# rgovindjee/mpconstellation

Measured on AMD Instinct MI355X. Metric: satellite-MPC-steps/sec (whole constellation; 1 step = discretize + constraint terms + solve per SCP iteration; inputs and results resident in HBM -- value_pcie is the same step with H2D of the inputs and D2H of the results inside), higher is better.
Workload: dtype f64

## Files before the change

mpconstellation_amd/csrc/solve_driver.hpp:

```cpp
#pragma once

#ifdef MPCX_WS_LDS
extern __shared__ double mpcx_ws_lds[];
#endif

namespace MPCX_NS {
#ifdef MPCX_PHASE_TIMING
#define PT_DECL unsigned long long pt_[12] = {0,0,0,0,0,0,0,0,0,0,0,0}, pt0_ = 0; unsigned pc_[12] = {0,0,0,0,0,0,0,0,0,0,0,0}; \
    const unsigned long long rt0_ = __builtin_amdgcn_s_memrealtime(), mt0_ = __builtin_amdgcn_s_memtime();
#define PT_BEGIN pt0_ = __builtin_amdgcn_s_memtime();
#define PT_END(i) { pt_[i] += __builtin_amdgcn_s_memtime() - pt0_; pc_[i]++; }
#else
#define PT_DECL
#define PT_BEGIN
#define PT_END(i)
#endif

#ifndef MPCX_SOLVE_WAVES
#define MPCX_SOLVE_WAVES 2
#endif

#ifndef MPCX_TP
__shared__ SatData g_sd;
__shared__ Scratch g_w;
// ... 65 lines not shown
    double v[GR_N];
    gr_clear(v);
    v[0] = r.sq; v[1] = r.zsum; v[2] = r.lsum; v[3] = r.prod_sum; v[4] = r.g_tf;
    v[GR_SUM] = r.dual_max; v[GR_SUM + 1] = r.prim_max; v[GR_SUM + 2] = r.prod_max;
    v[GR_SUM + GR_MAX] = r.prod_min;
    grid_reduce(g, v, lane);
    r.sq = v[0]; r.zsum = v[1]; r.lsum = v[2]; r.prod_sum = v[3]; r.g_tf = v[4];
    r.dual_max = v[GR_SUM]; r.prim_max = v[GR_SUM + 1]; r.prod_max = v[GR_SUM + 2]; r.prod_min = v[GR_SUM + GR_MAX];
    const double gtf = 1.0 + r.g_tf - gz[0] + gz[1];
    r.dual_max = fmax(r.dual_max, fabs(gtf)); r.sq += gtf * gtf;
    const double gv[2] = {-tf - b_tf[0], tf - b_tf[1]};
#pragma unroll
    for (int j = 0; j < 2; ++j) {
        const double pr = gv[j] + gs[j], sz = gs[j] * gz[j], q = sz - mu;
        r.prim_max = fmax(r.prim_max, fabs(pr)); r.sq += pr * pr + q * q;
        r.zsum += fabs(gz[j]); r.prod_min = fmin(r.prod_min, sz); r.prod_max = fmax(r.prod_max, sz); r.prod_sum += sz;
    }
}

template <bool SHARED>
__device__ __forceinline__ void solve_satellite(const SolveArgs &a, const int sat, const int slot, SatData &sd, Scratch &w, const int lane, GridSync *gsync = nullptr)
{
    PT_DECL
    const int Kmax = a.K;
    const int K = uni(a.Ks ? a.Ks[sat] : Kmax);
    if (K < 3 || K > Kmax) {
        cgf64 *xb = (cgf64 *)a.xbar + (size_t)sat * 7 * Kmax, *ub = (cgf64 *)a.ubar + (size_t)sat * 3 * Kmax;
        for (int e = lane; e < 7 * Kmax; e += 64) { a.X[(size_t)sat * 7 * Kmax + e] = xb[e]; a.NU[(size_t)sat * 7 * Kmax + e] = 0.0; }
        for (int e = lane; e < 3 * Kmax; e += 64) a.U[(size_t)sat * 3 * Kmax + e] = ub[e];
        if (lane == 0) {
            a.tf_out[sat] = (a.o.fixed_tf && !SHARED) ? 0.0 : a.tfbar[sat];
            a.status[sat] = MPCX_ST_BADK; a.iters[sat] = 0; a.kkt[sat] = 0.0;
            if (a.nreg) { a.nreg[2 * sat] = 0; a.nreg[2 * sat + 1] = -1; }
        }
        return;
    }
    { const Sat sv = sat_view(a, sat, slot, K, Kmax); if (lane == 0) g_s = sv; }
    WG_SYNC();
    Sat &s = g_s;
    const int KP = uni(s.KP);
    const SolveOpts &o = a.o;

    PT_BEGIN
    if (lane == 0) {
        double xK[7];
        for (int i = 0; i < 7; ++i) xK[i] = s.xbar[(size_t)i * Kmax + K - 1];
        build_terminal(xK, a.consts[(size_t)sat * MPCX_NCONST + MPCX_C_MU], a.r_des[sat], o, sd);
        sd.tfbar = a.tfbar[sat];
        double x0[3];
        for (int i = 0; i < 3; ++i) x0[i] = s.xbar[(size_t)i * Kmax];
        sd.infeas = structural_violation(x0, K, sd);
#ifdef MPCX_PHASE_TIMING
        for (int i = 0; i < 16; ++i) sd.fpt[i] = 0;
#endif
    }
    WG_SYNC();
    PT_END(11)
    PT_BEGIN
    double gr[GR_N];
    if (SHARED) {
        gr_clear(gr);
        gr[GR_SUM] = fmax(sd.infeas, -(sd.b_tf[0] + sd.b_tf[1]));
        grid_reduce(*gsync, gr, lane);
        if (lane == 0) sd.infeas = gsync->aborted ? 1.0 : gr[GR_SUM];
        WG_SYNC();
    }
    if (sd.infeas > 0.0) {
        for (int e = lane; e < 7 * Kmax; e += 64) { a.X[(size_t)sat * 7 * Kmax + e] = s.xbar[e]; a.NU[(size_t)sat * 7 * Kmax + e] = 0.0; }
        for (int e = lane; e < 3 * Kmax; e += 64) a.U[(size_t)sat * 3 * Kmax + e] = s.ubar[e];
        if (lane == 0) {
            if (!sd.fixed_tf || SHARED) a.tf_out[sat] = sd.tfbar; else a.tf_out[sat] = 0.0;
            a.status[sat] = (SHARED && gsync->aborted) ? MPCX_ST_NUMERIC : MPCX_ST_INFEASIBLE; a.iters[sat] = 0; a.kkt[sat] = sd.infeas;
            if (a.nreg) { a.nreg[2 * sat] = 0; a.nreg[2 * sat + 1] = -1; }
        }
        return;
    }
    {
        double *stg = (double *)&w;
        static_assert(sizeof(Scratch) >= 16 * MPCX_STAGE_DOUBLES * sizeof(double), "stage transposition buffer");
        for (int k0 = 0; k0 < K - 1; k0 += 16) {
            const int nk = (K - 1 - k0 < 16) ? K - 1 - k0 : 16;
            cgf64 *rec = s.A(k0);
            for (int e = lane; e < nk * MPCX_STAGE_DOUBLES; e += 64) stg[e] = rec[e];
            WG_SYNC();
            for (int e = lane; e < 16 * MPCX_STAGE_DOUBLES; e += 64) {
                const int f = e >> 4, kl = e & 15;
                if (kl < nk) s.stT[f * KP + k0 + kl] = stg[kl * MPCX_STAGE_DOUBLES + f];
            }
            WG_SYNC();
        }
    }
    PT_END(9)
    PT_BEGIN
    bool pushed = false;
    for (int k = lane; k < K; k += 64) {
        double x[7], u[3];
        for (int i = 0; i < 7; ++i) x[i] = s.xbar[(size_t)i * s.ldk + k];
        for (int i = 0; i < 3; ++i) u[i] = s.ubar[(size_t)i * s.ldk + k];
        const double rn = sqrt(x[0] * x[0] + x[1] * x[1] + x[2] * x[2]);
        const auto rb = s.rbn(k);
        for (int i = 0; i < 3; ++i) rb[i] = x[i] / rn;
        const auto p = s.itn(k);
        for (int i = 0; i < 7; ++i) { p[I_NU + i] = 0.0; p[I_LAM + i] = 0.0; }
        if (k == K - 1) for (int i = 0; i < 7; ++i) p[I_T + i] = 0.0;
        for (int i = 0; i < 7; ++i) p[I_X + i] = x[i];
        for (int i = 0; i < 3; ++i) p[I_U + i] = u[i];
// ... 276 lines not shown
            if (dec && cen) { have_trial = 1; break; }
            alpha = uni(alpha * 0.5);
        }
        if (!have_trial) {
            PT_BEGIN
            eval_residual<true>(s, sd, alpha, mu, mu_clip, lane);
            PT_END(10)
            if (SHARED) shared_trial();
        }
#ifdef MPCX_ITER_LOG
        if (lane == 0 && 5 * iter + 4 < 7 * K) { double *lg = a.X + (size_t)sat * 7 * Kmax + 5 * iter; lg[0] = mu; lg[1] = E0; lg[2] = alpha; lg[3] = delta_w; lg[4] = (double)fail_mask; }
#endif
        n_small = (alpha < kFbAlpha) ? n_small + 1 : 0;
        if (lane == 0) { wf64 *q = s.it; s.it = s.itB; s.itB = q; lf64 *g = s.itg; s.itg = s.itgB; s.itgB = g; }
        WG_SYNC();
        if (SHARED) { gs[0] = gst[0]; gs[1] = gst[1]; gz[0] = gzt[0]; gz[1] = gzt[1]; }
        {
            const double sq0 = rt.sq + 2.0 * mu * rt.prod_sum - (double)nzc * mu * mu;
            const ResAcc t = rt;
            WG_SYNC();
            r0 = t; r0.sq = sq0;
            WG_SYNC();
        }
    }

    for (int k = lane; k < K; k += 64) {
        const auto p = s.itn(k);
        for (int i = 0; i < 7; ++i) {
#ifndef MPCX_ITER_LOG
            a.X[(size_t)sat * 7 * Kmax + (size_t)i * Kmax + k] = p[I_X + i];
#endif
#if !(defined(MPCX_ITER_LOG) && defined(MPCX_LOG_IT))
            a.NU[(size_t)sat * 7 * Kmax + (size_t)i * Kmax + k] = (k <= K - 2) ? p[I_NU + i] : 0.0;
#endif
        }
#ifndef MPCX_ITER_LOG
        for (int i = 0; i < 3; ++i) a.U[(size_t)sat * 3 * Kmax + (size_t)i * Kmax + k] = p[I_U + i];
#endif
    }
    for (int k = K + lane; k < Kmax; k += 64) {
        for (int i = 0; i < 7; ++i) { a.X[(size_t)sat * 7 * Kmax + (size_t)i * Kmax + k] = 0.0; a.NU[(size_t)sat * 7 * Kmax + (size_t)i * Kmax + k] = 0.0; }
        for (int i = 0; i < 3; ++i) a.U[(size_t)sat * 3 * Kmax + (size_t)i * Kmax + k] = 0.0;
    }
    if (lane == 0) {
        a.tf_out[sat] = (sd.fixed_tf && !SHARED) ? r0.g_tf : s.itg[G_TF];
        a.status[sat] = status;
        a.iters[sat] = it_count;
        a.kkt[sat] = E0;
        if (a.nreg) { a.nreg[2 * sat] = n_reg; a.nreg[2 * sat + 1] = first_reg; }
#ifdef MPCX_PHASE_TIMING
        double *dbg = a.NU + (size_t)sat * 7 * Kmax;
        for (int i = 0; i < 12; ++i) { dbg[2 * i] = (double)pt_[i]; dbg[2 * i + 1] = (double)pc_[i]; }
        for (int i = 0; i < 16; ++i) dbg[24 + i] = (double)sd.fpt[i];
        dbg[40] = (double)(__builtin_amdgcn_s_memrealtime() - rt0_); dbg[41] = (double)(__builtin_amdgcn_s_memtime() - mt0_);
#ifdef MPCX_TP
        for (int i = 0; i < 16; ++i) dbg[48 + i] = (double)s.mail[16 + i];
#endif
#endif
    }
}

}
```

mpconstellation_amd/csrc/solve_phases.hpp:

```cpp
#pragma once

namespace MPCX_NS {
#ifdef MPCX_TWO_WAVE
using namespace mpcx;
#endif

struct ResAcc {
    double dual_max, prim_max, sq, zsum, lsum, prod_min, prod_max, prod_sum;
    double g_tf;
};

struct SatData {
    double aT[8][7], bT[8];
    int nT, linvt;
    int fixed_tf;
    int shared;
    double tS, rS;
    double w_vt, gh_vt, zeta_vt;
    double b_u, b_rmax, b_rmin, b_rfmax, b_tf[2], vt_des, w_tr, w_nu, tfbar;
    double WxK[49];
    double WxKsoft[49], gxKsoft[7];
    double ta[NTERM][7], tw[NTERM], tgh[NTERM], twin[NTERM];
    double avt[7], Hv[36], cv, gam, Wtf, gtf, sigmax;
    double Mb[NBD][NBD];
    double Sb[NBD][NBD];
    double siglam[NCH], xK[NCH][7];
    double sol[NBD];
    double zeta[NTERM];
    double red[8];
    double gl[3][GL_N];
    ResAcc racc[2];
    double rs_gtf, rs_rvt, rs_gex[NTERM];
    int dir_finite;
    struct Drv {
        double mu, dw_last, E0, delta_w, alpha, tau, mu_cur, rn0, mu_clip;
        int n_acc, status, it_count, n_reg, first_reg, mono, refined_prev, n_small, iter, have_dir, have_trial, clean, ls;
    } dv;
    double infeas;
    int flag;
#ifdef MPCX_PHASE_TIMING
    unsigned long long fpt[16];
#endif
};

__device__ __forceinline__ double relax(double b) { return b + kBoundRelax * fmax(1.0, fabs(b)); }

__device__ __forceinline__ double wave_max(double v)
{
#pragma unroll
    for (int o = 32; o > 0; o >>= 1) v = fmax(v, __shfl_xor(v, o, 64));
    return v;
}
__device__ __forceinline__ double wave_min(double v)
{
#pragma unroll
    for (int o = 32; o > 0; o >>= 1) v = fmin(v, __shfl_xor(v, o, 64));
    return v;
}
__device__ __forceinline__ double wave_sum(double v)
{
#pragma unroll
    for (int o = 32; o > 0; o >>= 1) v += __shfl_xor(v, o, 64);
    return v;
}

__device__ __forceinline__ double gshfl8(double v, int q)
{
    switch (q) {
    case 0: return bcast8<0>(v);
    case 1: return bcast8<1>(v);
    case 2: return bcast8<2>(v);
    case 3: return bcast8<3>(v);
    case 4: return bcast8<4>(v);
    case 5: return bcast8<5>(v);
    case 6: return bcast8<6>(v);
    default: return bcast8<7>(v);
    }
}

__device__ __forceinline__ void wsync()
{
    __builtin_amdgcn_fence(__ATOMIC_ACQ_REL, "wavefront");
    __builtin_amdgcn_wave_barrier();
}

__device__ __forceinline__ int uni(int v) { return __builtin_amdgcn_readfirstlane(v); }
__device__ __forceinline__ double uni(double v)
{
    const unsigned long long u = (unsigned long long)__double_as_longlong(v);
    const unsigned lo = __builtin_amdgcn_readfirstlane((unsigned)u), hi = __builtin_amdgcn_readfirstlane((unsigned)(u >> 32));
    return __longlong_as_double((long long)(((unsigned long long)hi << 32) | lo));
}

__device__ __forceinline__ double rcp_pos(double d)
{
    double r = __builtin_amdgcn_rcp(d);
#pragma unroll
    for (int n = 0; n < 2; ++n) { const double e = fma(-d, r, 1.0); r = fma(r, e, r); }
    return r;
}

__device__ void vt_reduced(const double *x, double vt_des, double &c, double *g6, double *H36)
{
    const double *r = x, *v = x + 3;
    const double q = r[0] * r[0] + r[1] * r[1] + r[2] * r[2];
    const double rv = r[0] * v[0] + r[1] * v[1] + r[2] * v[2];
    const double iq = 1.0 / q, iq2 = iq * iq, iq3 = iq2 * iq;
    c = v[0] * v[0] + v[1] * v[1] + v[2] * v[2] - rv * rv * iq - vt_des * vt_des;
    if (!g6) return;
    for (int i = 0; i < 3; ++i) {
        g6[i] = -2.0 * rv * v[i] * iq + 2.0 * rv * rv * r[i] * iq2;
        g6[3 + i] = 2.0 * v[i] - 2.0 * rv * r[i] * iq;
    }
    if (!H36) return;
    for (int i = 0; i < 3; ++i)
        for (int j = 0; j < 3; ++j) {
            const double I = (i == j) ? 1.0 : 0.0;
            const double Hvv = 2.0 * I - 2.0 * r[i] * r[j] * iq;
            const double Hrr = -2.0 * v[i] * v[j] * iq + 4.0 * rv * (v[i] * r[j] + r[i] * v[j]) * iq2 +
                               2.0 * rv * rv * I * iq2 - 8.0 * rv * rv * r[i] * r[j] * iq3;
            const double Hrv = -2.0 * v[i] * r[j] * iq - 2.0 * rv * I * iq + 4.0 * rv * r[i] * r[j] * iq2;
            H36[i * 6 + j] = Hrr;
            H36[(3 + i) * 6 + 3 + j] = Hvv;
            H36[i * 6 + 3 + j] = Hrv;
            H36[(3 + j) * 6 + i] = Hrv;
        }
}

__device__ __noinline__ void build_terminal(const double *xK, double mu_grav, double r_des, const SolveOpts &o, SatData &sd)
{
    double r[3] = {xK[0], xK[1], xK[2]}, v[3] = {xK[3], xK[4], xK[5]}, h[3], rh[3], hh[3];
    const double rn = sqrt(r[0] * r[0] + r[1] * r[1] + r[2] * r[2]);
    h[0] = r[1] * v[2] - r[2] * v[1]; h[1] = r[2] * v[0] - r[0] * v[2]; h[2] = r[0] * v[1] - r[1] * v[0];
    const double hn = sqrt(h[0] * h[0] + h[1] * h[1] + h[2] * h[2]);
    for (int i = 0; i < 3; ++i) { rh[i] = r[i] / rn; hh[i] = h[i] / hn; }
    const double ihn = 1.0 / hn, ihn3 = 1.0 / (hn * hn * hn), irn = 1.0 / rn, irn3 = 1.0 / (rn * rn * rn);
    double Ph[9], hh3[9], nSv[9], Sr[9], Dr_h[9], Dv_h[9], Dr_r[9];
    for (int i = 0; i < 3; ++i)
        for (int j = 0; j < 3; ++j) {
// ... 350 lines not shown
#pragma unroll
                for (int j = 0; j < 3; ++j) { bn[j] = Bn[i * 3 + j]; bp[j] = Bp[i * 3 + j]; bm[j] = Bm[i * 3 + j]; }
                const double sg = Sg[i], xv = xi[i];
                const double nu0 = p[I_NU + i], dnu_ = d[I_NU + i], tt0 = p[I_T + i], lam = TRIAL(p, d, I_LAM + i);
                const double stp0 = p[I_STP + i], ztp0 = p[I_ZTP + i], stn0 = p[I_STN + i], ztn0 = p[I_ZTN + i];
                const double xn = TRIAL(pn, dn, I_X + i);
                const double lmv = TRIAL(pm, dm, I_LAM + i);
                const double dnu = z ? 0.0 : dnu_;
                const L1Dir ld = l1_dir(nu0, tt0, stp0, ztp0, stn0, ztn0, dnu, mu, w_nu);
                const bool lon = !z && dyn;
                const double nu = fma(a, dnu, nu0), tt = fma(a, lon ? ld.dt : 0.0, tt0);
                double stp = fma(a, lon ? ld.dstp : 0.0, stp0), ztp = fma(a, lon ? ld.dztp : 0.0, ztp0);
                double stn = fma(a, lon ? ld.dstn : 0.0, stn0), ztn = fma(a, lon ? ld.dztn : 0.0, ztn0);
                if (WRITE && dyn) { POST(stp, ztp, nu - tt); POST(stn, ztn, -nu - tt); }
                const double lm = (valid && has_prev) ? lmv : 0.0;
                gx[r] += half ? 0.0 : lm; gx[(4 + r) % 7] += (half && valid) ? lm : 0.0;
#pragma unroll
                for (int j = 0; j < 3; ++j) gu[j] -= bm[j] * lm;
                if (valid && dyn) {
                    double acc = sg * tf + xv + nu;
#pragma unroll
                    for (int j = 0; j < 7; ++j) acc += ar[j] * x[j];
#pragma unroll
                    for (int j = 0; j < 3; ++j) acc += bn[j] * u[j] + bp[j] * un[j];
                    ACC_P(xn - acc);
                    nsv[NS_E + i] = xn - acc;
                    sl += sg * lam;
                    lsum += fabs(lam);
                    ACC_D(ztp - ztn - lam);
                    ACC_D(w_nu - ztp - ztn);
                    ACC_P(nu - tt + stp);
                    ACC_P(-nu - tt + stn);
                    ACC_C(stp, ztp);
                    ACC_C(stn, ztn);
#pragma unroll
                    for (int j = 0; j < 7; ++j) gx[j] -= ar[j] * lam;
#pragma unroll
                    for (int j = 0; j < 3; ++j) gu[j] -= bn[j] * lam;
                }
                if (WRITE && valid) {
                    w[I_NU + i] = nu; w[I_T + i] = tt; w[I_LAM + i] = lam;
                    w[I_STP + i] = stp; w[I_ZTP + i] = ztp; w[I_STN + i] = stn; w[I_ZTN + i] = ztn;
                }
                CHUNK_END
            }
            gtf_part -= sl;
        }
#pragma unroll
        for (int i = 0; i < 7; ++i) gx[i] += __shfl_xor(gx[i], 32, 64);
#pragma unroll
        for (int i = 0; i < 3; ++i) gu[i] += __shfl_xor(gu[i], 32, 64);
        if (h0) {
            if (k == K - 1) {
                if (!sd.linvt) {
                    double cv, g6[6];
                    vt_reduced(x, sd.vt_des, cv, g6, nullptr);
                    ACC_P(cv);
#pragma unroll
                    for (int i = 0; i < 6; ++i) gx[i] += lvt * g6[i];
                    lsum += fabs(lvt);
                }
                const int nT = sd.nT;
                for (int j = 0; j < nT; ++j) {
                    const int js = gs_term(j), jz = gz_term(j);
                    double sj = s.itg[js] + a * s.drg[js];
                    double zj = s.itg[jz] + a * s.drg[jz];
                    double gj = -sd.bT[j];
                    for (int i = 0; i < 7; ++i) gj += sd.aT[j][i] * x[i];
                    if (WRITE) { POST(sj, zj, gj); s.itgB[js] = sj; s.itgB[jz] = zj; }
                    for (int i = 0; i < 7; ++i) gx[i] += sd.aT[j][i] * zj;
                    ACC_P(gj + sj);
                    ACC_C(sj, zj);
                }
                double srf = s.itg[G_SRF] + a * s.drg[G_SRF], zrf = s.itg[G_ZRF] + a * s.drg[G_ZRF];
                const double g_rf = x[0] * x[0] + x[1] * x[1] + x[2] * x[2] - sd.b_rfmax;
                if (WRITE) { POST(srf, zrf, g_rf); s.itgB[G_SRF] = srf; s.itgB[G_ZRF] = zrf; s.itgB[G_LVT] = lvt; }
                ACC_P(g_rf + srf);
                ACC_C(srf, zrf);
                for (int i = 0; i < 3; ++i) gx[i] += 2.0 * x[i] * zrf;
            }
            if (has_prev) {
#pragma unroll
                for (int i = 0; i < 7; ++i) ACC_D(gx[i]);
            }
#pragma unroll
            for (int i = 0; i < 3; ++i) ACC_D(gu[i]);
        }
    }
    double gtf = wave_sum(gtf_part);
    out.g_tf = gtf + 2.0 * sd.w_tr * (tf - sd.tfbar);
    if (lane == 0 && sd.fixed_tf) {
        if (WRITE) s.itgB[G_TF] = tf;
    } else if (lane == 0) {
        double s0 = s.itg[G_STF] + a * s.drg[G_STF], s1 = s.itg[G_STF + 1] + a * s.drg[G_STF + 1];
        double z0 = s.itg[G_ZTF] + a * s.drg[G_ZTF], z1 = s.itg[G_ZTF + 1] + a * s.drg[G_ZTF + 1];
        if (WRITE) {
            POST(s0, z0, -tf - sd.b_tf[0]); POST(s1, z1, tf - sd.b_tf[1]);
            s.itgB[G_TF] = tf; s.itgB[G_STF] = s0; s.itgB[G_STF + 1] = s1; s.itgB[G_ZTF] = z0; s.itgB[G_ZTF + 1] = z1;
        }
        gtf += 1.0 + 2.0 * sd.w_tr * (tf - sd.tfbar) - z0 + z1;
        ACC_D(gtf);
        ACC_P(-tf - sd.b_tf[0] + s0);
        ACC_P(tf - sd.b_tf[1] + s1);
        ACC_C(s0, z0);
        ACC_C(s1, z1);
    }
#undef ACC_D
#undef ACC_P
#undef ACC_C
#undef TRIAL
#undef POST
    out.dual_max = wave_max(dual); out.prim_max = wave_max(prim);
    out.sq = wave_sum(sq); out.zsum = wave_sum(zsum); out.lsum = wave_sum(lsum);
    out.prod_min = wave_min(pmin); out.prod_max = wave_max(pmax); out.prod_sum = wave_sum(psum);
    WG_SYNC();
}

__device__ __forceinline__ int n_ineq(int K, int nT, int fixed_tf) { return K + (K - 1) + (K - 2) + nT + 1 + 14 * (K - 1) + (fixed_tf ? 0 : 2); }

__device__ double scaled_error_n(const ResAcc &r, int nz, int nl, double mu)
{
    const double smax = 100.0;
    const double sdl = fmax(smax, (r.zsum + r.lsum) / (double)(nz + nl)) / smax;
    const double sc = fmax(smax, r.zsum / (double)nz) / smax;
    const double comp = fmax(r.prod_max - mu, mu - r.prod_min);
    return fmax(fmax(r.dual_max / sdl, r.prim_max), comp / sc);
}
__device__ double scaled_error(const ResAcc &r, int K, int nT, int fixed_tf, double mu)
{
    const double smax = 100.0;
    const int nz = n_ineq(K, nT, fixed_tf), nl = 7 * (K - 1) + (nT == 6 ? 1 : 0);
    const double sdl = fmax(smax, (r.zsum + r.lsum) / (double)(nz + nl)) / smax;
    const double sc = fmax(smax, r.zsum / (double)nz) / smax;
    const double comp = fmax(r.prod_max - mu, mu - r.prod_min);
    return fmax(fmax(r.dual_max / sdl, r.prim_max), comp / sc);
}

template <bool KEEP_NS>
__device__ __noinline__ void newton_blocks(const Sat &s, SatData &sd, double *stg, double mu, double delta_w, int lane)
{
    const int K = s.K;
    const double w_tr = sd.w_tr, w_nu = sd.w_nu, b_u = sd.b_u, b_rmax = sd.b_rmax, b_rmin = sd.b_rmin;
    const int half = HALF_OF(lane);
    const bool h0 = (half == 0);
    double sigmax = 0.0;
    for (int k0 = 0; k0 < K; k0 += 32) {
      const int k = k0 + NODE_OF(lane);
      if (k < K) {
        const auto p = s.itn(k);
        const auto ns = s.nsn(k);
        const auto rb = s.rbn(k);
        double *nb = stg + NODE_OF(lane) * NB_N;
        double *rhs = stg + 32 * NB_N + NODE_OF(lane) * RHS_LD;
        const bool dyn = (k <= K - 2), inner = (k >= 1 && k <= K - 2);
        double x[7], u[3], gx[7], gu[3], Wx3[9];
        double zh_rmax = 0.0, sig_rmax = 0.0, zrmax;
        double rv[4][7];
        {
// ... 62 lines not shown
                        Wx3[i * 3 + j] += (i == j ? 2.0 * zrmax : 0.0) + in_max * 4.0 * x[i] * x[j] + in_min * rbv[i] * rbv[j];
                }
            }
            if (h0) {
#pragma unroll
                for (int i = 0; i < 9; ++i) nb[N_WU + i] = Wu[i];
                if (!inner) { nb[N_SX + SX_EX] = 0.0; nb[N_SX + SX_A] = 0.0; nb[N_SX + SX_A + 1] = 0.0; nb[N_SX + SX_A + 2] = 0.0; }
                if (KEEP_NS) {
#pragma unroll
                    for (int i = 0; i < 7; ++i) ns[NS_GX + i] = gx[i];
#pragma unroll
                    for (int i = 0; i < 3; ++i) ns[NS_GU + i] = gu[i];
                }
#pragma unroll
                for (int i = 0; i < 3; ++i) rhs[R_GU + i] = gu[i];
                if (k != K - 1) {
#pragma unroll
                    for (int i = 0; i < 7; ++i) rhs[R_GX + i] = (k == 0) ? 0.0 : gx[i];
                }
            }
            if (h0 && k != K - 1) {
#pragma unroll
                for (int i = 0; i < 9; ++i) nb[N_W3 + i] = Wx3[i];
                nb[N_DIAG] = 2.0 * w_tr + delta_w; nb[N_ZERO] = 0.0;
            }
        }
        CHUNK_END
        {
#pragma unroll
            for (int r = 0; r < 4; ++r) {
                const int iv = 4 * half + r;
                const bool valid = (iv < 7) && dyn;
                const int i = (iv < 7) ? iv : 6;
                const double nu = rv[r][0], tt = rv[r][1], stp = rv[r][2], ztp = rv[r][3];
                const double stn = rv[r][4], ztn = rv[r][5];
                const double g1 = nu - tt, g2 = -nu - tt;
                const double ip = rcp_pos(stp), in = rcp_pos(stn);
                const double s1 = ztp * ip, s2 = ztn * in;
                const double zh1 = mu * ip + s1 * (g1 + stp), zh2 = mu * in + s2 * (g2 + stn);
                const double aa = s1 + s2, bb = s2 - s1, gt = w_nu - zh1 - zh2;
                const double ia = rcp_pos(aa);
                const double dd = 4.0 * s1 * s2 * ia;
                const double ek = rv[r][6];
                const double rho = (zh1 - zh2) - (bb * ia) * gt;
                if (valid) {
                    nb[N_D + i] = dd;
                    if (KEEP_NS) { ns[NS_D + i] = dd; ns[NS_RHO + i] = rho; }
                }
                if (iv < 7) { rhs[R_RHO + i] = dyn ? rho : 0.0; rhs[R_AFF + i] = dyn ? -ek : 0.0; }
            }
            CHUNK_END
        }
        if (h0 && k == K - 1) {
            double g6[6];
            const double lvt = sd.linvt ? 0.0 : s.itg[G_LVT];
            double sig[8], zh[8];
#pragma unroll
            for (int j = 0; j < 8; ++j) {
                sig[j] = 0.0; zh[j] = 0.0;
                if (j >= sd.nT) continue;
                double gj = -sd.bT[j];
                for (int i = 0; i < 7; ++i) gj += sd.aT[j][i] * x[i];
                const double sj = s.itg[gs_term(j)], zj = s.itg[gz_term(j)];
                sig[j] = zj / sj; zh[j] = mu / sj + sig[j] * (gj + sj);
            }
            if (!sd.linvt) {
                double cv;
                vt_reduced(x, sd.vt_des, cv, g6, sd.Hv);
                sd.cv = cv;
            } else {
                for (int i = 0; i < 6; ++i) g6[i] = sd.aT[6][i];
                for (int i = 0; i < 36; ++i) sd.Hv[i] = 0.0;
                sd.cv = 0.0;
                sd.w_vt = sig[6] + sig[7]; sd.gh_vt = zh[6] - zh[7];
            }
            for (int i = 0; i < 7; ++i) sd.avt[i] = (i < 6) ? g6[i] : 0.0;
            const double srf = s.itg[G_SRF], zrf = s.itg[G_ZRF];
            const double grf = x[0] * x[0] + x[1] * x[1] + x[2] * x[2] - sd.b_rfmax;
            const double sigrf = zrf / srf, zhrf = mu / srf + sigrf * (grf + srf);
            sd.red[0] = 2.0 * (zrmax + zrf);
            sd.red[1] = lvt;
            for (int i = 0; i < 7; ++i) sd.gxKsoft[i] = gx[i];
            const int rows[NTERM] = {0, 1, 3, 5, -1};
            for (int t = 0; t < NTERM; ++t) {
                if (rows[t] >= 0) for (int i = 0; i < 7; ++i) sd.ta[t][i] = sd.aT[rows[t]][i];
                else for (int i = 0; i < 7; ++i) sd.ta[t][i] = (i < 3) ? 2.0 * x[i] : 0.0;
            }
            sd.tw[0] = sig[0]; sd.tgh[0] = zh[0];
            sd.tw[1] = sig[1] + sig[2]; sd.tgh[1] = zh[1] - zh[2];
            sd.tw[2] = sig[3] + sig[4]; sd.tgh[2] = zh[3] - zh[4];
            sd.tw[3] = sig[5]; sd.tgh[3] = zh[5];
            sd.tw[4] = sig_rmax + sigrf; sd.tgh[4] = zh_rmax + zhrf;
            for (int t = 0; t < NTERM; ++t) sd.twin[t] = fmin(sd.tw[t], kTermCap);
            double hn = 0.0, an = 0.0;
            for (int i = 0; i < 36; ++i) hn += sd.Hv[i] * sd.Hv[i];
            for (int i = 0; i < 6; ++i) an += g6[i] * g6[i];
            sd.gam = sd.linvt ? fmin(sd.w_vt, kTermCap) : (kTermCap + 10.0 * fabs(lvt) * sqrt(hn)) / an;
            {
                const double rvt = sd.linvt ? -sd.gh_vt / sd.w_vt : -sd.cv;
                double gK[7];
                for (int i = 0; i < 7; ++i) gK[i] = gx[i];
                for (int t = 0; t < NTERM; ++t) {
                    const double share = (sd.tw[t] > 0.0) ? sd.twin[t] / sd.tw[t] : 1.0;
                    for (int i = 0; i < 7; ++i) gK[i] += sd.tgh[t] * share * sd.ta[t][i];
                }
                for (int i = 0; i < 7; ++i) rhs[R_GX + i] = gK[i] - sd.gam * rvt * sd.avt[i];
            }
#pragma unroll
            for (int i = 0; i <= N_ZERO; ++i) nb[i] = 0.0;
        }
      }
      WG_SYNC();
      {
          const int ne = ((K - k0 < 32) ? K - k0 : 32) * NB_N;
          wf64 *dst = s.nb + (size_t)k0 * NB_N;
          for (int e = lane; e < ne; e += 64) dst[e] = stg[e];
          const int nr = ((K - k0 < 32) ? K - k0 : 32) * RHS_N;
          wf64 *ch = s.ch + (size_t)k0 * CH_N + C_RHS;
          for (int e = lane; e < nr; e += 64) { const int kl = e / RHS_N, i = e - kl * RHS_N; ch[(size_t)kl * CH_N + i] = stg[32 * NB_N + kl * RHS_LD + i]; }
      }
      WG_SYNC();
    }
    sigmax = wave_max(sigmax);
    WG_SYNC();
    if (lane < 49) {
        const int i = lane / 7, j = lane - 7 * i;
        double soft = (i == j) ? 2.0 * w_tr + delta_w + (i < 3 ? sd.red[0] : 0.0) : 0.0;
        if (i < 6 && j < 6) soft += sd.red[1] * sd.Hv[i * 6 + j];
        double full = soft;
#pragma unroll
        for (int t = 0; t < NTERM; ++t) full += sd.twin[t] * sd.ta[t][i] * sd.ta[t][j];
        full += sd.gam * sd.avt[i] * sd.avt[j];
        sd.WxKsoft[lane] = soft; sd.WxK[lane] = full;
    }
    if (lane == 0 && sd.shared) {
        sd.Wtf = 2.0 * sd.w_tr; sd.gtf = 2.0 * sd.w_tr * (s.itg[G_TF] - sd.tfbar); sd.sigmax = sigmax;
    } else if (lane == 0 && sd.fixed_tf) { sd.Wtf = 1.0; sd.gtf = 0.0; sd.sigmax = sigmax; }
    else if (lane == 0) {
        const double tf = s.itg[G_TF];
        double W = 2.0 * sd.w_tr + delta_w, g = 1.0 + 2.0 * sd.w_tr * (tf - sd.tfbar);
        const double gv[2] = {-tf - sd.b_tf[0], tf - sd.b_tf[1]};
        for (int j = 0; j < 2; ++j) {
            const double sj = s.itg[G_STF + j], zj = s.itg[G_ZTF + j];
            const double sig = zj / sj, zh = mu / sj + sig * (gv[j] + sj);
            W += sig; g += (j == 0 ? -zh : zh);
            sigmax = fmax(sigmax, sig);
        }
        sd.Wtf = W; sd.gtf = g; sd.sigmax = sigmax;
    }
    WG_SYNC();
}

__device__ __noinline__ void combine_channels(const Sat &s_in, SatData &sd, double *stg, int lane, bool first)
{
    const Sat s = uniform_view(s_in);
    const int K = s.K, KP = s.KP;
    double sol[NBD];
#pragma unroll
    for (int j = 0; j < NBD; ++j) sol[j] = sd.sol[j];
    wf64 *dr = wave_uniform(s.dr);
    cwf64 *it = wave_uniform((cwf64 *)s.it);
    cgf64 *traj = wave_uniform((cgf64 *)s.traj);
    for (int k0 = 0; k0 < K; k0 += 32) {
        const int nk = (K - k0 < 32) ? K - k0 : 32;
        const int n = nk * TR_N;
        constexpr int CQ = 8;
        for (int e0 = 0; e0 < n; e0 += 64 * CQ) {
            double v[CQ];
            int slot[CQ];
#pragma unroll
            for (int q = 0; q < CQ; ++q) {
                const int e = e0 + 64 * q + lane;
                const int ec = (e < n) ? e : 0;
                const int kl = ec / TR_N, i = ec - kl * TR_N;
                cgf64 *tr = traj + (size_t)(k0 + kl) * NCH * TR_N + i;
                double acc = tr[0];
#pragma unroll
                for (int j = 0; j < NBD; ++j)
                    acc += sol[j] * tr[(1 + j) * TR_N];
                v[q] = acc; slot[q] = (e < n) ? i * CMB_LD + kl : -1;
            }
#pragma unroll
            for (int q = 0; q < CQ; ++q) if (slot[q] >= 0) stg[slot[q]] = v[q];
        }
        WG_SYNC();
        constexpr int NQ = DIR_N * 32 / 64;
        double curv[NQ], Dv[NQ], rv[NQ];
#pragma unroll
        for (int q = 0; q < NQ; ++q) {
            const int e = lane + 64 * q;
            const int i = e >> 5, kl = e & 31, k = k0 + kl;
            const int off = (i < T_U) ? I_X + i : (i < T_NU ? I_U + (i - T_U) : (i < T_LAM ? I_NU + (i - T_NU) : I_LAM + (i - T_LAM)));
            const int dst = off * KP + (kl < nk ? k : k0);
            const int kc = (kl < nk) ? k : k0, j = (i >= T_LAM) ? i - T_LAM : 0;
            curv[q] = first ? it[dst] : dr[dst];
            Dv[q] = s.nb[(size_t)kc * NB_N + N_D + j]; rv[q] = s.ch[(size_t)kc * CH_N + C_RHS + R_RHO + j];
        }
        CHUNK_END
#pragma unroll
        for (int q = 0; q < NQ; ++q) {
            const int e = lane + 64 * q;
            const int i = e >> 5, kl = e & 31, k = k0 + kl;
            const bool act = kl < nk && !(k == K - 1 && i >= T_NU);
            const int off = (i < T_U) ? I_X + i : (i < T_NU ? I_U + (i - T_U) : (i < T_LAM ? I_NU + (i - T_NU) : I_LAM + (i - T_LAM)));
            const int dst = off * KP + (kl < nk ? k : k0);
            const double cur = curv[q];
            const double base = first ? ((i >= T_LAM) ? -cur : 0.0) : cur;
            const int j = (i >= T_LAM) ? i - T_LAM : 0;
            const double val = (i >= T_LAM) ? fma(Dv[q], stg[(T_NU + j) * CMB_LD + kl], rv[q]) : stg[(i < T_LAM ? i : 0) * CMB_LD + kl];
            if (act) dr[dst] = base + val;
        }
        WG_SYNC();
    }
    if (lane == 0) {
        if (first) { s.drg[G_TF] = sd.sol[0]; s.drg[G_LVT] = sd.linvt ? 0.0 : -s.itg[G_LVT] + sd.sol[1]; }
        else { s.drg[G_TF] += sd.sol[0]; if (!sd.linvt) s.drg[G_LVT] += sd.sol[1]; }
        if (sd.linvt) sd.zeta_vt = (first ? 0.0 : sd.zeta_vt) + sd.sol[1];
        for (int t = 0; t < NTERM; ++t) sd.zeta[t] = (first ? 0.0 : sd.zeta[t]) + sd.sol[2 + t];
    }
    WG_SYNC();
}

__device__ __noinline__ void reduced_residual(const Sat &s, SatData &sd, double *stg, int lane)
{
    double rvt_rhs, gex[NTERM];
    const int K = s.K;
    double gtf_part = 0.0;
    const double dtf = s.drg[G_TF];
    double gin[NTERM], rvt_x;
    {
        const auto dKc = s.drn(K - 1);
        double dK[7];
#pragma unroll
        for (int i = 0; i < 7; ++i) dK[i] = dKc[I_X + i];
        double av = 0.0;
#pragma unroll
        for (int i = 0; i < 7; ++i) av += sd.avt[i] * dK[i];
        rvt_rhs = -sd.cv - av;
        rvt_x = rvt_rhs;
        if (sd.linvt) {
            const double wex = sd.w_vt - sd.gam;
            const bool on = wex > 0.0;
            rvt_x = -(sd.gh_vt * (sd.gam / sd.w_vt) + sd.gam * av + (on ? sd.zeta_vt : 0.0)) / sd.gam;
            rvt_rhs = on ? -(av - sd.zeta_vt / wex + sd.gh_vt / sd.w_vt) : 0.0;
        }
        for (int t = 0; t < NTERM; ++t) {
            double adx = 0.0;
#pragma unroll
            for (int i = 0; i < 7; ++i) adx += sd.ta[t][i] * dK[i];
            const double wex = sd.tw[t] - sd.twin[t];
            const double share = (sd.tw[t] > 0.0) ? sd.twin[t] / sd.tw[t] : 1.0;
            const bool on = wex > 0.0;
            gin[t] = sd.tgh[t] * share + sd.twin[t] * adx + (on ? sd.zeta[t] : 0.0);
            gex[t] = on ? (adx - sd.zeta[t] / wex + sd.tgh[t] / sd.tw[t]) * wex : 0.0;
        }
    }
    for (int k0 = 0; k0 < K; k0 += 64) {
      const int k = k0 + lane;
      double *rec = stg + lane * RHS_LD;
      if (k < K) {
        cwf64 *nb = s.nb + (size_t)k * NB_N;
        const auto ns = s.nsn(k);
        const auto p = s.itn(k), d = s.drn(k);
        const bool hp = (k >= 1), dyn = (k <= K - 2), term = (k == K - 1);
        const auto pm = p.node(hp ? -1 : 0), dm = d.node(hp ? -1 : 0), dn = d.node(dyn ? 1 : 0);
        double lt[7], ltm[7];
#pragma unroll
        for (int i = 0; i < 7; ++i) {
            const double a0 = p[I_LAM + i], a1 = d[I_LAM + i], b0 = pm[I_LAM + i], b1 = dm[I_LAM + i];
            lt[i] = dyn ? a0 + a1 : 0.0;
            ltm[i] = hp ? b0 + b1 : 0.0;
        }
        CHUNK_END
        double dx[7], du[3], dnu[7], nsgx[7], nsgu[3], w3[9], wu[9], sx[SX_N];
#pragma unroll
        for (int i = 0; i < 7; ++i) { dx[i] = d[I_X + i]; dnu[i] = d[I_NU + i]; nsgx[i] = ns[NS_GX + i]; }
#pragma unroll
        for (int i = 0; i < 3; ++i) { du[i] = d[I_U + i]; nsgu[i] = ns[NS_GU + i]; }
#pragma unroll
        for (int i = 0; i < 9; ++i) { w3[i] = nb[N_W3 + i]; wu[i] = nb[N_WU + i]; }
#pragma unroll
        for (int i = 0; i < SX_N; ++i) sx[i] = nb[N_SX + i];
        const double dg = nb[N_DIAG];
        CHUNK_END
        double gx[7], gu[3];
        if (hp) {
            if (term) {
#pragma unroll
                for (int i = 0; i < 7; ++i) {
                    double acc = sd.gxKsoft[i] + ltm[i];
#pragma unroll
                    for (int j = 0; j < 7; ++j) acc += sd.WxKsoft[i * 7 + j] * dx[j];
                    gx[i] = acc;
                }
            } else {
#pragma unroll
                for (int i = 0; i < 7; ++i) {
                    double acc = nsgx[i] + ltm[i];
                    if (i < 3) {
#pragma unroll
                        for (int j = 0; j < 3; ++j) acc += w3[i * 3 + j] * dx[j];
                    } else acc += dg * dx[i];
                    gx[i] = acc;
                }
            }
            if (term) {
                const double lvt = s.itg[G_LVT] + s.drg[G_LVT];
#pragma unroll
// ... 163 lines not shown
#pragma unroll
        for (int i = 0; i < 7; ++i) { x[i] = p[I_X + i]; dx[i] = d[I_X + i]; }
#pragma unroll
        for (int i = 0; i < 3; ++i) { u[i] = p[I_U + i]; du[i] = d[I_U + i]; }
#pragma unroll
        for (int i = 0; i < 6; ++i) bs[i] = p[I_SU + i];
        const double rb0 = rb[0], rb1 = rb[1], rb2 = rb[2];
#pragma unroll
        for (int r = 0; r < 4; ++r) {
            const int iv = 4 * half + r;
            const int i = (iv < 7) ? iv : 6;
            rv[r][0] = p[I_NU + i]; rv[r][1] = p[I_T + i]; rv[r][2] = p[I_STP + i]; rv[r][3] = p[I_ZTP + i];
            rv[r][4] = p[I_STN + i]; rv[r][5] = p[I_ZTN + i]; rv[r][6] = d[I_NU + i]; rv[r][7] = d[I_LAM + i];
        }
        CHUNK_END
        {
#pragma unroll
            for (int i = 0; i < 7; ++i) CHK(dx[i]);
#pragma unroll
            for (int i = 0; i < 3; ++i) CHK(du[i]);
            {
                const PairDir q = pair_dir(bs[0], bs[1], u[0] * u[0] + u[1] * u[1] + u[2] * u[2] - b_u,
                                           2.0 * (u[0] * du[0] + u[1] * du[1] + u[2] * du[2]), mu);
                LIM(bs[0], q.ds); LIM(bs[1], q.dz);
            }
            if (k >= 1) {
                const PairDir q = pair_dir(bs[2], bs[3], x[0] * x[0] + x[1] * x[1] + x[2] * x[2] - b_rmax,
                                           2.0 * (x[0] * dx[0] + x[1] * dx[1] + x[2] * dx[2]), mu);
                LIM(bs[2], q.ds); LIM(bs[3], q.dz);
            }
            if (k >= 1 && k <= K - 2) {
                const PairDir q = pair_dir(bs[4], bs[5], -(rb0 * x[0] + rb1 * x[1] + rb2 * x[2]) - b_rmin,
                                           -(rb0 * dx[0] + rb1 * dx[1] + rb2 * dx[2]), mu);
                LIM(bs[4], q.ds); LIM(bs[5], q.dz);
            }
        }
        {
            const bool dyn = (k <= K - 2);
#pragma unroll
            for (int r = 0; r < 4; ++r) {
                const int iv = 4 * half + r;
                const bool valid = (iv < 7) && dyn;
                const double nu = rv[r][0], tt = rv[r][1], stp = rv[r][2], ztp = rv[r][3];
                const double stn = rv[r][4], ztn = rv[r][5], dnu = rv[r][6], dlam = rv[r][7];
                const L1Dir q = l1_dir(nu, tt, stp, ztp, stn, ztn, dnu, mu, w_nu);
                if (valid) {
                    CHK(dnu); CHK(dlam); CHK(q.dt);
                    LIM(stp, q.dstp); LIM(ztp, q.dztp);
                    LIM(stn, q.dstn); LIM(ztn, q.dztn);
                }
            }
        }
        if (h0 && k == K - 1) {
            for (int j = 0; j < sd.nT; ++j) {
                const int js = gs_term(j), jz = gz_term(j);
                double gj = -sd.bT[j], dg = 0.0;
                for (int i = 0; i < 7; ++i) { gj += sd.aT[j][i] * x[i]; dg += sd.aT[j][i] * dx[i]; }
                const double sj = s.itg[js], zj = s.itg[jz];
                const double sig = zj / sj, zh = mu / sj + sig * (gj + sj);
                s.drg[js] = -(gj + sj) - dg; s.drg[jz] = zh + sig * dg - zj;
                LIM(sj, s.drg[js]); LIM(zj, s.drg[jz]);
            }
            const double srf = s.itg[G_SRF], zrf = s.itg[G_ZRF];
            const double g = x[0] * x[0] + x[1] * x[1] + x[2] * x[2] - sd.b_rfmax;
            const double sig = zrf / srf, zh = mu / srf + sig * (g + srf);
            const double dg = 2.0 * (x[0] * dx[0] + x[1] * dx[1] + x[2] * dx[2]);
            s.drg[G_SRF] = -(g + srf) - dg; s.drg[G_ZRF] = zh + sig * dg - zrf;
            LIM(srf, s.drg[G_SRF]); LIM(zrf, s.drg[G_ZRF]);
        }
    }
    if (lane == 0 && !sd.fixed_tf) {
        const double tf = s.itg[G_TF], dtf = s.drg[G_TF];
        const double gv[2] = {-tf - sd.b_tf[0], tf - sd.b_tf[1]}, dgv[2] = {-dtf, dtf};
        for (int j = 0; j < 2; ++j) {
            const double sj = s.itg[G_STF + j], zj = s.itg[G_ZTF + j];
            const double sig = zj / sj, zh = mu / sj + sig * (gv[j] + sj);
            s.drg[G_STF + j] = -(gv[j] + sj) - dgv[j]; s.drg[G_ZTF + j] = zh + sig * dgv[j] - zj;
            LIM(sj, s.drg[G_STF + j]); LIM(zj, s.drg[G_ZTF + j]);
        }
    }
    if (!(fabs(s.drg[G_TF]) < 1e300)) bad = 1.0;
#undef LIM
#undef CHK
    amax = wave_min(amax);
    sd.dir_finite = (wave_max(bad) == 0.0) ? 1 : 0;
    WG_SYNC();
    return amax;
}

}
```

Before: 738,600.

## Spread terminal-constraint rows across lanes in residual and direction recovery

The terminal-node constraint work (up to 8 linear terminal rows, the radius constraint and two tf bounds) was done serially by one lane. It now runs across 11 lanes: the owning lane stages x, gradient and step vectors in shared SatData.tx, and each lane handles one constraint row. Results are gathered back with readlane broadcasts and the gradient fold is spread over 7 lanes. Optional phase-timing counters are also added. The cost is extra wave syncs, shared staging and readlane traffic.

Result: no change. 738,500 (-0.0%).

```diff
diff --git a/mpconstellation_amd/csrc/solve_driver.hpp b/mpconstellation_amd/csrc/solve_driver.hpp
--- a/mpconstellation_amd/csrc/solve_driver.hpp
+++ b/mpconstellation_amd/csrc/solve_driver.hpp
@@ -141,6 +141,7 @@
         sd.infeas = structural_violation(x0, K, sd);
 #ifdef MPCX_PHASE_TIMING
         for (int i = 0; i < 16; ++i) sd.fpt[i] = 0;
+        for (int i = 0; i < 8; ++i) sd.olt[i] = 0;
 #endif
     }
     WG_SYNC();
@@ -523,6 +524,7 @@
         double *dbg = a.NU + (size_t)sat * 7 * Kmax;
         for (int i = 0; i < 12; ++i) { dbg[2 * i] = (double)pt_[i]; dbg[2 * i + 1] = (double)pc_[i]; }
         for (int i = 0; i < 16; ++i) dbg[24 + i] = (double)sd.fpt[i];
+        if (7 * Kmax >= 72) for (int i = 0; i < 8; ++i) dbg[64 + i] = (double)sd.olt[i];
         dbg[40] = (double)(__builtin_amdgcn_s_memrealtime() - rt0_); dbg[41] = (double)(__builtin_amdgcn_s_memtime() - mt0_);
 #ifdef MPCX_TP
         for (int i = 0; i < 16; ++i) dbg[48 + i] = (double)s.mail[16 + i];
diff --git a/mpconstellation_amd/csrc/solve_phases.hpp b/mpconstellation_amd/csrc/solve_phases.hpp
--- a/mpconstellation_amd/csrc/solve_phases.hpp
+++ b/mpconstellation_amd/csrc/solve_phases.hpp
@@ -10,6 +10,7 @@
     double g_tf;
 };
 
+constexpr int TROWS = 11;
 struct SatData {
     double aT[8][7], bT[8];
     int nT, linvt;
@@ -28,6 +29,7 @@
     double sol[NBD];
     double zeta[NTERM];
     double red[8];
+    double tx[17];
     double gl[3][GL_N];
     ResAcc racc[2];
     double rs_gtf, rs_rvt, rs_gex[NTERM];
@@ -40,8 +42,17 @@
     int flag;
 #ifdef MPCX_PHASE_TIMING
     unsigned long long fpt[16];
+    unsigned long long olt[8];
 #endif
 };
+
+#ifdef MPCX_PHASE_TIMING
+#define OL_BEGIN const unsigned long long ol0_ = __builtin_amdgcn_s_memtime();
+#define OL_END(i) { sd.olt[i] += __builtin_amdgcn_s_memtime() - ol0_; }
+#else
+#define OL_BEGIN
+#define OL_END(i)
+#endif
 
 __device__ __forceinline__ double relax(double b) { return b + kBoundRelax * fmax(1.0, fabs(b)); }
 
@@ -85,6 +96,12 @@
 }
 
 __device__ __forceinline__ int uni(int v) { return __builtin_amdgcn_readfirstlane(v); }
+__device__ __forceinline__ double lane_value(double v, int l)
+{
+    const unsigned long long u = (unsigned long long)__double_as_longlong(v);
+    const unsigned lo = __builtin_amdgcn_readlane((unsigned)u, l), hi = __builtin_amdgcn_readlane((unsigned)(u >> 32), l);
+    return __longlong_as_double((long long)(((unsigned long long)hi << 32) | lo));
+}
 __device__ __forceinline__ double uni(double v)
 {
     const unsigned long long u = (unsigned long long)__double_as_longlong(v);
@@ -541,58 +558,104 @@
         for (int i = 0; i < 3; ++i) gu[i] += __shfl_xor(gu[i], 32, 64);
         if (h0) {
             if (k == K - 1) {
-                if (!sd.linvt) {
-                    double cv, g6[6];
-                    vt_reduced(x, sd.vt_des, cv, g6, nullptr);
-                    ACC_P(cv);
-#pragma unroll
-                    for (int i = 0; i < 6; ++i) gx[i] += lvt * g6[i];
-                    lsum += fabs(lvt);
-                }
-                const int nT = sd.nT;
-                for (int j = 0; j < nT; ++j) {
-                    const int js = gs_term(j), jz = gz_term(j);
-                    double sj = s.itg[js] + a * s.drg[js];
-                    double zj = s.itg[jz] + a * s.drg[jz];
-                    double gj = -sd.bT[j];
-                    for (int i = 0; i < 7; ++i) gj += sd.aT[j][i] * x[i];
-                    if (WRITE) { POST(sj, zj, gj); s.itgB[js] = sj; s.itgB[jz] = zj; }
-                    for (int i = 0; i < 7; ++i) gx[i] += sd.aT[j][i] * zj;
-                    ACC_P(gj + sj);
-                    ACC_C(sj, zj);
-                }
-                double srf = s.itg[G_SRF] + a * s.drg[G_SRF], zrf = s.itg[G_ZRF] + a * s.drg[G_ZRF];
-                const double g_rf = x[0] * x[0] + x[1] * x[1] + x[2] * x[2] - sd.b_rfmax;
-                if (WRITE) { POST(srf, zrf, g_rf); s.itgB[G_SRF] = srf; s.itgB[G_ZRF] = zrf; s.itgB[G_LVT] = lvt; }
-                ACC_P(g_rf + srf);
-                ACC_C(srf, zrf);
-                for (int i = 0; i < 3; ++i) gx[i] += 2.0 * x[i] * zrf;
-            }
-            if (has_prev) {
-#pragma unroll
-                for (int i = 0; i < 7; ++i) ACC_D(gx[i]);
-            }
-#pragma unroll
-            for (int i = 0; i < 3; ++i) ACC_D(gu[i]);
+#pragma unroll
+                for (int i = 0; i < 7; ++i) { sd.tx[i] = x[i]; sd.tx[7 + i] = gx[i]; }
+#pragma unroll
+                for (int i = 0; i < 3; ++i) sd.tx[14 + i] = gu[i];
+            } else {
+                if (has_prev) {
+#pragma unroll
+                    for (int i = 0; i < 7; ++i) ACC_D(gx[i]);
+                }
+#pragma unroll
+                for (int i = 0; i < 3; ++i) ACC_D(gu[i]);
+            }
         }
     }
     double gtf = wave_sum(gtf_part);
     out.g_tf = gtf + 2.0 * sd.w_tr * (tf - sd.tfbar);
-    if (lane == 0 && sd.fixed_tf) {
-        if (WRITE) s.itgB[G_TF] = tf;
-    } else if (lane == 0) {
-        double s0 = s.itg[G_STF] + a * s.drg[G_STF], s1 = s.itg[G_STF + 1] + a * s.drg[G_STF + 1];
-        double z0 = s.itg[G_ZTF] + a * s.drg[G_ZTF], z1 = s.itg[G_ZTF + 1] + a * s.drg[G_ZTF + 1];
+    wsync();
+    {
+        OL_BEGIN
+        const int nT = uni(sd.nT);
+        const bool linvt = uni(sd.linvt) != 0, fixed_tf = uni(sd.fixed_tf) != 0;
+        const int own = (K - 1) & 31;
+        double x[7];
+#pragma unroll
+        for (int i = 0; i < 7; ++i) x[i] = sd.tx[i];
+        const int rr = (lane < TROWS) ? lane : 8, r8 = rr & 7;
+        const int js = rr < 8 ? gs_term(rr) : (rr == 8 ? G_SRF : G_STF + (rr - 9));
+        const int jz = rr < 8 ? gz_term(rr) : (rr == 8 ? G_ZRF : G_ZTF + (rr - 9));
+        const bool act = (rr == lane) && (rr < 8 ? rr < nT : (rr == 8 || !fixed_tf));
+        double sj = s.itg[js] + a * s.drg[js];
+        double zj = s.itg[jz] + a * s.drg[jz];
+        double gj = -sd.bT[r8];
+#pragma unroll
+        for (int i = 0; i < 7; ++i) gj += sd.aT[r8][i] * x[i];
+        const double g_rf = x[0] * x[0] + x[1] * x[1] + x[2] * x[2] - sd.b_rfmax;
+        const double g_t0 = -tf - sd.b_tf[0], g_t1 = tf - sd.b_tf[1];
+        const double g = rr < 8 ? gj : (rr == 8 ? g_rf : (rr == 9 ? g_t0 : g_t1));
         if (WRITE) {
-            POST(s0, z0, -tf - sd.b_tf[0]); POST(s1, z1, tf - sd.b_tf[1]);
-            s.itgB[G_TF] = tf; s.itgB[G_STF] = s0; s.itgB[G_STF + 1] = s1; s.itgB[G_ZTF] = z0; s.itgB[G_ZTF + 1] = z1;
-        }
-        gtf += 1.0 + 2.0 * sd.w_tr * (tf - sd.tfbar) - z0 + z1;
-        ACC_D(gtf);
-        ACC_P(-tf - sd.b_tf[0] + s0);
-        ACC_P(tf - sd.b_tf[1] + s1);
-        ACC_C(s0, z0);
-        ACC_C(s1, z1);
+            POST(sj, zj, g);
+            if (act) { s.itgB[js] = sj; s.itgB[jz] = zj; }
+            if (lane == 0) { s.itgB[G_TF] = tf; s.itgB[G_LVT] = lvt; }
+        }
+        const double qp = g + sj, pr = sj * zj;
+        if (act) { prim = fmax(prim, fabs(qp)); pmin = fmin(pmin, pr); pmax = fmax(pmax, pr); }
+        double cv = 0.0, g6[6] = {0.0, 0.0, 0.0, 0.0, 0.0, 0.0};
+        if (!linvt) vt_reduced(x, sd.vt_des, cv, g6, nullptr);
+        double ts[TROWS], tz[TROWS], tp[TROWS];
+#pragma unroll
+        for (int j = 0; j < TROWS; ++j) { ts[j] = lane_value(sj, j); tz[j] = lane_value(zj, j); tp[j] = lane_value(qp, j); }
+        double tg[7];
+        {
+            const int ci = (lane < 7) ? lane : 0;
+            double gxi = sd.tx[7 + ci];
+            const double xi = sd.tx[ci < 3 ? ci : 0];
+            double ac[8];
+#pragma unroll
+            for (int j = 0; j < 8; ++j) ac[j] = sd.aT[j][ci];
+            if (!linvt) {
+                double g6i = 0.0;
+#pragma unroll
+                for (int i = 0; i < 6; ++i) g6i = (ci == i) ? g6[i] : g6i;
+                gxi = (ci < 6) ? gxi + lvt * g6i : gxi;
+            }
+#pragma unroll
+            for (int j = 0; j < 8; ++j) gxi = (j < nT) ? gxi + ac[j] * tz[j] : gxi;
+            gxi = (ci < 3) ? gxi + 2.0 * xi * tz[8] : gxi;
+            if (lane < 7 && K >= 2) dual = fmax(dual, fabs(gxi));
+#pragma unroll
+            for (int i = 0; i < 7; ++i) tg[i] = lane_value(gxi, i);
+        }
+        double tu[3];
+#pragma unroll
+        for (int i = 0; i < 3; ++i) tu[i] = sd.tx[14 + i];
+#define FOLD_P(v) { const double q_ = (v); sq += q_ * q_; }
+#define FOLD_C(sv, zv) { const double s_ = (sv), z_ = (zv), q_ = s_ * z_ - mu; sq += q_ * q_; zsum += fabs(z_); psum += s_ * z_; }
+        if (lane == own) {
+            if (!linvt) { ACC_P(cv); lsum += fabs(lvt); }
+#pragma unroll
+            for (int j = 0; j < 9; ++j)
+                if (j == 8 || j < nT) { FOLD_P(tp[j]); FOLD_C(ts[j], tz[j]); }
+            if (K >= 2) {
+#pragma unroll
+                for (int i = 0; i < 7; ++i) FOLD_P(tg[i]);
+            }
+#pragma unroll
+            for (int i = 0; i < 3; ++i) ACC_D(tu[i]);
+        }
+        if (lane == 0 && !fixed_tf) {
+            gtf += 1.0 + 2.0 * sd.w_tr * (tf - sd.tfbar) - tz[9] + tz[10];
+            ACC_D(gtf);
+            FOLD_P(tp[9]);
+            FOLD_P(tp[10]);
+            FOLD_C(ts[9], tz[9]);
+            FOLD_C(ts[10], tz[10]);
+        }
+#undef FOLD_P
+#undef FOLD_C
+        OL_END(0)
     }
 #undef ACC_D
 #undef ACC_P
@@ -761,6 +824,7 @@
             CHUNK_END
         }
         if (h0 && k == K - 1) {
+            OL_BEGIN
             double g6[6];
             const double lvt = sd.linvt ? 0.0 : s.itg[G_LVT];
             double sig[8], zh[8];
@@ -817,6 +881,7 @@
             }
 #pragma unroll
             for (int i = 0; i <= N_ZERO; ++i) nb[i] = 0.0;
+            OL_END(2)
         }
       }
       WG_SYNC();
@@ -846,6 +911,7 @@
         sd.Wtf = 2.0 * sd.w_tr; sd.gtf = 2.0 * sd.w_tr * (s.itg[G_TF] - sd.tfbar); sd.sigmax = sigmax;
     } else if (lane == 0 && sd.fixed_tf) { sd.Wtf = 1.0; sd.gtf = 0.0; sd.sigmax = sigmax; }
     else if (lane == 0) {
+        OL_BEGIN
         const double tf = s.itg[G_TF];
         double W = 2.0 * sd.w_tr + delta_w, g = 1.0 + 2.0 * sd.w_tr * (tf - sd.tfbar);
         const double gv[2] = {-tf - sd.b_tf[0], tf - sd.b_tf[1]};
@@ -856,6 +922,7 @@
             sigmax = fmax(sigmax, sig);
         }
         sd.Wtf = W; sd.gtf = g; sd.sigmax = sigmax;
+        OL_END(3)
     }
     WG_SYNC();
 }
@@ -922,10 +989,12 @@
         WG_SYNC();
     }
     if (lane == 0) {
+        OL_BEGIN
         if (first) { s.drg[G_TF] = sd.sol[0]; s.drg[G_LVT] = sd.linvt ? 0.0 : -s.itg[G_LVT] + sd.sol[1]; }
         else { s.drg[G_TF] += sd.sol[0]; if (!sd.linvt) s.drg[G_LVT] += sd.sol[1]; }
         if (sd.linvt) sd.zeta_vt = (first ? 0.0 : sd.zeta_vt) + sd.sol[1];
         for (int t = 0; t < NTERM; ++t) sd.zeta[t] = (first ? 0.0 : sd.zeta[t]) + sd.sol[2 + t];
+        OL_END(4)
     }
     WG_SYNC();
 }
@@ -938,6 +1007,7 @@
     const double dtf = s.drg[G_TF];
     double gin[NTERM], rvt_x;
     {
+        OL_BEGIN
         const auto dKc = s.drn(K - 1);
         double dK[7];
 #pragma unroll
@@ -963,6 +1033,7 @@
             gin[t] = sd.tgh[t] * share + sd.twin[t] * adx + (on ? sd.zeta[t] : 0.0);
             gex[t] = on ? (adx - sd.zeta[t] / wex + sd.tgh[t] / sd.tw[t]) * wex : 0.0;
         }
+        OL_END(7)
     }
     for (int k0 = 0; k0 < K; k0 += 64) {
       const int k = k0 + lane;
@@ -1232,33 +1303,41 @@
             }
         }
         if (h0 && k == K - 1) {
-            for (int j = 0; j < sd.nT; ++j) {
-                const int js = gs_term(j), jz = gz_term(j);
-                double gj = -sd.bT[j], dg = 0.0;
-                for (int i = 0; i < 7; ++i) { gj += sd.aT[j][i] * x[i]; dg += sd.aT[j][i] * dx[i]; }
-                const double sj = s.itg[js], zj = s.itg[jz];
-                const double sig = zj / sj, zh = mu / sj + sig * (gj + sj);
-                s.drg[js] = -(gj + sj) - dg; s.drg[jz] = zh + sig * dg - zj;
-                LIM(sj, s.drg[js]); LIM(zj, s.drg[jz]);
-            }
-            const double srf = s.itg[G_SRF], zrf = s.itg[G_ZRF];
-            const double g = x[0] * x[0] + x[1] * x[1] + x[2] * x[2] - sd.b_rfmax;
-            const double sig = zrf / srf, zh = mu / srf + sig * (g + srf);
-            const double dg = 2.0 * (x[0] * dx[0] + x[1] * dx[1] + x[2] * dx[2]);
-            s.drg[G_SRF] = -(g + srf) - dg; s.drg[G_ZRF] = zh + sig * dg - zrf;
-            LIM(srf, s.drg[G_SRF]); LIM(zrf, s.drg[G_ZRF]);
-        }
-    }
-    if (lane == 0 && !sd.fixed_tf) {
+#pragma unroll
+            for (int i = 0; i < 7; ++i) { sd.tx[i] = x[i]; sd.tx[7 + i] = dx[i]; }
+        }
+    }
+    wsync();
+    {
+        OL_BEGIN
+        const int nT = uni(sd.nT);
+        const bool fixed_tf = uni(sd.fixed_tf) != 0;
+        double x[7], dx[7];
+#pragma unroll
+        for (int i = 0; i < 7; ++i) { x[i] = sd.tx[i]; dx[i] = sd.tx[7 + i]; }
+        const int rr = (lane < TROWS) ? lane : 8, r8 = rr & 7;
+        const int js = rr < 8 ? gs_term(rr) : (rr == 8 ? G_SRF : G_STF + (rr - 9));
+        const int jz = rr < 8 ? gz_term(rr) : (rr == 8 ? G_ZRF : G_ZTF + (rr - 9));
+        const bool act = (rr == lane) && (rr < 8 ? rr < nT : (rr == 8 || !fixed_tf));
+        const double sj = s.itg[js], zj = s.itg[jz];
         const double tf = s.itg[G_TF], dtf = s.drg[G_TF];
+        double gj = -sd.bT[r8], dgj = 0.0;
+#pragma unroll
+        for (int i = 0; i < 7; ++i) { gj += sd.aT[r8][i] * x[i]; dgj += sd.aT[r8][i] * dx[i]; }
+        const double g_rf = x[0] * x[0] + x[1] * x[1] + x[2] * x[2] - sd.b_rfmax;
+        const double dg_rf = 2.0 * (x[0] * dx[0] + x[1] * dx[1] + x[2] * dx[2]);
         const double gv[2] = {-tf - sd.b_tf[0], tf - sd.b_tf[1]}, dgv[2] = {-dtf, dtf};
-        for (int j = 0; j < 2; ++j) {
-            const double sj = s.itg[G_STF + j], zj = s.itg[G_ZTF + j];
-            const double sig = zj / sj, zh = mu / sj + sig * (gv[j] + sj);
-            s.drg[G_STF + j] = -(gv[j] + sj) - dgv[j]; s.drg[G_ZTF + j] = zh + sig * dgv[j] - zj;
-            LIM(sj, s.drg[G_STF + j]); LIM(zj, s.drg[G_ZTF + j]);
-        }
-    }
+        const double g = rr < 8 ? gj : (rr == 8 ? g_rf : gv[rr == 9 ? 0 : 1]);
+        const double dg = rr < 8 ? dgj : (rr == 8 ? dg_rf : dgv[rr == 9 ? 0 : 1]);
+        const double sig = zj / sj, zh = mu / sj + sig * (g + sj);
+        const double ds = -(g + sj) - dg, dz = zh + sig * dg - zj;
+        if (act) {
+            s.drg[js] = ds; s.drg[jz] = dz;
+            LIM(sj, ds); LIM(zj, dz);
+        }
+        OL_END(5)
+    }
+    wsync();
     if (!(fabs(s.drg[G_TF]) < 1e300)) bad = 1.0;
 #undef LIM
 #undef CHK
```
